# pedrosecchi67/ImmersedBoundary.jl

Hardware: AMD Instinct MI355X
Metric: Mcells*iters/s residual sweep (advection-JST-MUSCL), 2D RAE2822 (higher is better)
Workload: dtype f32

## Files before the change

### immersedboundary.jl_amd/csrc/ibh_quad2d.h

```cpp
#pragma once
#include "ibh_sweep2d.h"

namespace quad2 {

#pragma clang fp contract(fast)

typedef float v2f __attribute__((ext_vector_type(2)));
typedef float v4f __attribute__((ext_vector_type(4)));
typedef int v2i __attribute__((ext_vector_type(2)));
typedef float v4f_g __attribute__((ext_vector_type(4), aligned(4)));

#define QUAD_PITCH 20
#define QUAD_TILE (16 * QUAD_PITCH)
#define QUAD_OFF_EXT (4 * QUAD_TILE)
#define QUAD_OFF_RING (QUAD_OFF_EXT + 160)
#define QUAD_OFF_EX (QUAD_OFF_RING + 3 * 64)
#define QUAD_LDS (QUAD_OFF_EX + 64)

__device__ __forceinline__ float dpp_shr1(float old, float v) {
    return __int_as_float(__builtin_amdgcn_update_dpp(__float_as_int(old), __float_as_int(v), 0x111, 0xf, 0xf, false));
}
__device__ __forceinline__ float dpp_shl1(float old, float v) {
    return __int_as_float(__builtin_amdgcn_update_dpp(__float_as_int(old), __float_as_int(v), 0x101, 0xf, 0xf, false));
}
__device__ __forceinline__ float dpp_shl1z(float v) {
    return __int_as_float(__builtin_amdgcn_update_dpp(0, __float_as_int(v), 0x101, 0xf, 0xf, true));
}
__device__ __forceinline__ float bperm(int byte_addr, float v) {
    return __int_as_float(__builtin_amdgcn_ds_bpermute(byte_addr, __float_as_int(v)));
}
__device__ __forceinline__ float max3(float a, float b, float c) { return fmaxf(fmaxf(a, b), c); }
__device__ __forceinline__ float lds_read(const float* p) {
    float v = *p;
    asm volatile("" : "+v"(v));
    return v;
}

__device__ __forceinline__ v4f flux_half4(v4f ua, v4f ub, v4f Sa, v4f Sb, v4f Da, v4f Db, v4f Ca, v4f Cb) {
    const v4f d = ub - ua;
    const v4f gu = Sa - 0.5f * d;
    const v4f Du = Sb - 0.5f * d;
    v4f s, Df;
#pragma unroll
    for (int c = 0; c < 4; ++c) {
        s[c] = __builtin_amdgcn_fmed3f(Du[c], gu[c], 0.0f);
        Df[c] = max3(Da[c], Db[c], 1e-7f);
    }
    const v4f t16 = (Sa - Sb) * 0.0625f;
    const v4f uf = (ua + 0.5f * d) + t16;
    const v4f A = uf - Df * t16;
    const v4f Cf = 0.5f * (Ca + Cb);
    const v4f B = Df * (s - 0.5f * d);
    const v4f CA = Cf * A;
    v4f F;
#pragma unroll
    for (int c = 0; c < 4; ++c) F[c] = fmaf(fabsf(Cf[c]), B[c], CA[c]);
    return F;
}

__device__ __forceinline__ v2f flux_w2(float ua, v2f ub, float Sa, v2f Sb, float Da, v2f Db, float Ca, v2f Cb, float wa) {
    const v2f d = ub - ua;
    const v2f gu = Sa - d * wa;
    const v2f Du = Sb - d * (1.0f - wa);
    const v2f s = v2f{__builtin_amdgcn_fmed3f(Du.x, gu.x, 0.0f), __builtin_amdgcn_fmed3f(Du.y, gu.y, 0.0f)};
    const v2f t16 = (Sa - Sb) * 0.0625f;
    const v2f uf = (ua + wa * d) + t16;
    const v2f mu = d * (0.5f - wa) - t16;
    const v2f Df = v2f{max3(Da, Db.x, 1e-7f), max3(Da, Db.y, 1e-7f)};
    const v2f A = uf + Df * mu;
    const v2f Cf = Ca + wa * (Cb - Ca);
    const v2f B = Df * (s - 0.5f * d);
    const v2f CA = Cf * A;
    return v2f{fmaf(fabsf(Cf.x), B.x, CA.x), fmaf(fabsf(Cf.y), B.y, CA.y)};
}

__device__ __forceinline__ float jst(float g, float a, float rh) {
    return fmaf(fabsf(g), rh, 1e-7f) * __builtin_amdgcn_rcpf(fmaf(a, rh, 1e-7f));
}
__device__ __forceinline__ float jst_max2(float g1, float a1, float rh1, float g2, float a2, float rh2) {
    const float n1 = fmaf(fabsf(g1), rh1, 1e-7f), d1 = fmaf(a1, rh1, 1e-7f);
    const float n2 = fmaf(fabsf(g2), rh2, 1e-7f), d2 = fmaf(a2, rh2, 1e-7f);
    return fmaxf(fmaxf(n1 * d2, n2 * d1) * __builtin_amdgcn_rcpf(d1 * d2), 1e-7f);
}

template <bool HALF>
struct QuadLaneTab {
    uint32_t w[64][8];
    constexpr QuadLaneTab() : w() {
        for (int lane = 0; lane < 64; ++lane) {
            const int g = lane >> 4, t = lane & 15, tl = lane & 7, lhs = lane >> 3;
            const int ytop = HALF ? 7 : 15;
            const bool g0 = g == 0, g3 = g == 3, lr = g0 || g3, t0 = t == 0, t15 = t == ytop;
            const int bx = g0 ? 0 : g3 ? 15 : t, by = lr ? t : g == 1 ? 0 : ytop;
            const int pos_b = by * QUAD_PITCH + bx;
            const int pos_b1 = lr ? (t ^ 1) * QUAD_PITCH + bx : by * QUAD_PITCH + (t ^ 1);
            const int pos_own = t * QUAD_PITCH + 4 * g;
            const int myrow = t0 ? 0 : t15 ? 1 : 2, rowB = t0 ? 0 : 2, rowT = t15 ? 1 : 2;
            const int wrow = g == 1 ? 0 : g == 2 ? 1 : 3;
            const int eline = (lane & 31) >> 2, ee = lane & 3;
            const int epos = QUAD_OFF_EXT + eline * 20 + (ee < 2 ? ee : 16 + ee);
            const int line = QUAD_OFF_EXT + lhs * 20;
            const uint32_t f[14] = {
                (uint32_t)pos_own, (uint32_t)pos_b, (uint32_t)pos_b1, (uint32_t)(line + 2 + 2 * tl), (uint32_t)epos,
                (uint32_t)(QUAD_OFF_RING + wrow * 16 + t), (uint32_t)(QUAD_OFF_RING + myrow * 16 + 4 * g),
                (uint32_t)(QUAD_OFF_RING + rowB * 16 + 4 * g), (uint32_t)(QUAD_OFF_RING + rowT * 16 + 4 * g),
                (uint32_t)(line + 2 * tl), (uint32_t)(line + 2 * (tl & ~1)), (uint32_t)(line + 2 * (tl | 1) + 4),
                0u, 0u};
            for (int k = 0; k < 6; ++k) w[lane][k] = (4u * f[2 * k]) | ((4u * f[2 * k + 1]) << 16);
            w[lane][6] = 64u * ((g >> 1) + 2 * (t >> 3)) + 4u * (g & 1) + 8u * (t & 7);
            w[lane][7] = (uint32_t)(g0 ? -1 : g == 1 ? -8 : g == 2 ? 8 : 1);
        }
    }
};
__device__ const QuadLaneTab<false> lane_tab = QuadLaneTab<false>();
__device__ const QuadLaneTab<true> lane_tab_half = QuadLaneTab<true>();

struct QuadLane {
    float *p_own;
    float *p_b;
    float *p_b1;
    float *p_extw;
    float *p_epos;
    float *p_ringw;
    float *p_ringm;
    float *p_ringB;
    float *p_ringT;
    float *p_LbS;
    float *p_LbC;
    float *p_HbC;
    uint32_t a0off;
    int delta;
    int lane, tl, lhs;
    bool g0, g3, lr, dny, t15;
    bool active;
    float sgn;
};

template <bool HALF = false>
__device__ __forceinline__ QuadLane quad_lane(float* lds, int lane) {
    QuadLane G;
    char* const L = (char*)lds;
    const uint32_t* const tab = HALF ? lane_tab_half.w[lane] : lane_tab.w[lane];
    const uint4 w0 = *(const uint4*)(tab);
    const uint4 w1 = *(const uint4*)(tab + 4);
#define QL_LO(w) ((w) & 0xffffu)
#define QL_HI(w) ((w) >> 16)
    G.p_own = (float*)(L + QL_LO(w0.x));
    G.p_b = (float*)(L + QL_HI(w0.x));
    G.p_b1 = (float*)(L + QL_LO(w0.y));
    G.p_extw = (float*)(L + QL_HI(w0.y));
    G.p_epos = (float*)(L + QL_LO(w0.z));
    G.p_ringw = (float*)(L + QL_HI(w0.z));
    G.p_ringm = (float*)(L + QL_LO(w0.w));
    G.p_ringB = (float*)(L + QL_HI(w0.w));
    G.p_ringT = (float*)(L + QL_LO(w1.x));
    G.p_LbS = (float*)(L + QL_HI(w1.x));
    G.p_LbC = (float*)(L + QL_LO(w1.y));
    G.p_HbC = (float*)(L + QL_HI(w1.y));
#undef QL_LO
#undef QL_HI
    G.a0off = ((lane & 7) << 3) | (HALF ? 0 : ((lane & 8) << 4)) | ((lane & 16) >> 2) | ((lane & 32) << 1);
    G.delta = (int)w1.w;
    G.lane = lane;
    G.tl = lane & 7;
    G.lhs = lane >> 3;
    G.g0 = lane < 16;
    G.g3 = lane >= 48;
    G.lr = G.g0 || G.g3;
    G.dny = !G.lr;
    G.t15 = (lane & 15) == (HALF ? 7 : 15);
    G.active = !HALF || (lane & 8) == 0;
    G.sgn = lane >= 32 ? 1.0f : -1.0f;
    ((float*)(L + 4 * (QUAD_OFF_RING + 64 + 32)))[lane & 15] = 0.0f;
    ((float*)(L + 4 * (QUAD_OFF_RING + 128 + 32)))[lane & 15] = 0.5f;
    return G;
}

struct QuadTab {
    QuadDesc2 d;
    v2i hid;
    uint32_t eid;
};
struct QuadOwn {
    v4f U, CX, CY;
    uint32_t a0;
};
struct QuadHalo {
    v2f hu, hd, hc;
    float eu;
};
__device__ __forceinline__ QuadTab quad_load_tab(const QuadDesc2* __restrict__ qd, const int32_t* __restrict__ qtab,
                                                 int32_t q, int lane, const int32_t* __restrict__ qaux = nullptr) {
    QuadTab T;
    T.d = qd[q];
    const int32_t* row = qtab + (size_t)q * IBH_QROW;
    if (qaux) {
        const int32_t* aux = qaux + (size_t)q * IBH_QAUX;
        const int lhs = lane >> 3, tl = lane & 7;
        const int32_t orig = aux[32 + lhs];
        T.eid = (uint32_t)aux[lane & 31];
        const bool isC = ((T.d.cls >> (4 * lhs)) & 15u) == SIDE_COARSE;
        const bool lr = lane < 16 || lane >= 48;
        const int32_t id = orig + (lr ? 8 : 1) * (isC ? tl >> 1 : tl);
        T.hid = v2i{id, id};
        if (orig < 0) T.hid = *(const v2i*)(row + 2 * lane);
        return T;
    }
    T.hid = *(const v2i*)(row + 2 * lane);
    T.eid = (uint32_t)row[128 + (lane & 31)];
    return T;
}
__device__ __forceinline__ QuadOwn quad_load_own(const QuadLane& G, const QuadTab& T, const float* __restrict__ u,
                                                 const float* __restrict__ C, uint32_t ldc) {
    QuadOwn O;
    O.a0 = (uint32_t)T.d.base + G.a0off;
    O.U = *(const v4f_g*)((const char*)u + ((size_t)O.a0 << 2));
    O.CX = *(const v4f_g*)((const char*)C + ((size_t)O.a0 << 2));
    O.CY = *(const v4f_g*)((const char*)(C + ldc) + ((size_t)O.a0 << 2));
    return O;
}
__device__ __forceinline__ QuadHalo quad_load_halo_paired(const QuadLane& G, const QuadTab& T, const float* __restrict__ u,
                                                          const float* __restrict__ C, uint32_t ldc) {
    using blk2::ldg;
    typedef float v2f_g __attribute__((ext_vector_type(2), aligned(4)));
    auto pair = [](const float* p, int i) { return *(const v2f_g*)((const char*)p + ((size_t)(uint32_t)i << 2)); };
    QuadHalo H;
    const float* Cn = C + (G.dny ? ldc : 0u);
    const bool isF = ((T.d.cls >> (4 * G.lhs)) & 15u) == SIDE_FINE;
    const int lo = G.delta < 0 ? G.delta : 0;
    const v2f PA = pair(u, G.lr ? T.hid.x + lo : T.hid.x);
    const v2f PB = pair(u, G.lr ? T.hid.y + lo : T.hid.x + G.delta);
    const v2f PC = pair(Cn, T.hid.x);
    H.eu = ldg(u, T.eid);
    float hc1 = 0.0f;
    if (G.lr && isF) hc1 = ldg(Cn, (uint32_t)T.hid.y);
    asm volatile("" : "+v"(hc1));
    const bool first = G.g0;
    const float huA = first ? PA.y : PA.x, hdA = first ? PA.x : PA.y;
    const float huB = first ? PB.y : PB.x, hdB = first ? PB.x : PB.y;
    H.hu.x = G.lr ? huA : PA.x;
    H.hd.x = G.lr ? hdA : PB.x;
    H.hu.y = G.lr ? huB : (isF ? PA.y : PA.x);
    H.hd.y = G.lr ? hdB : (isF ? PB.y : PB.x);
    H.hc.x = PC.x;
    H.hc.y = isF ? (G.lr ? hc1 : PC.y) : PC.x;
    return H;
}

template <bool STAMP, bool STEP = false, bool HALF = false>
__device__ __forceinline__ void quad_compute(const QuadLane& G, const QuadTab& T, const QuadOwn& O, const QuadHalo& H,
                                             float* __restrict__ ud, unsigned long long* stamps, float dt = 0.0f) {
    using blk2::wave_lds_sync;
    auto stamp = [&](int k) {
        if constexpr (STAMP) {
            __builtin_amdgcn_s_waitcnt(0);
            if (stamps && G.lane == 0) stamps[k] = __builtin_amdgcn_s_memrealtime();
        }
    };
    const v4f U = O.U, CX = O.CX, CY = O.CY;
    const v2f hu = H.hu, hd = H.hd, hc = H.hc;
    const bool g0 = G.g0, g3 = G.g3, lr = G.lr, dny = G.dny, t15 = G.t15;
    const int lane = G.lane;
    const float sgn = G.sgn;
    const uint32_t ty = (T.d.cls >> (4 * G.lhs)) & 15u;
    const bool isC = ty == SIDE_COARSE, isF = ty == SIDE_FINE;
    const float qs = isC ? (1.0f / 3.0f) : isF ? (2.0f / 3.0f) : 0.5f;
    const float irt = isC ? 0.5f : isF ? 2.0f : 1.0f;
    const float rhx = T.d.rh[0], rhy = T.d.rh[1];

    *(v4f*)G.p_own = U;
    *(v4f*)(G.p_own + 3 * QUAD_TILE) = CY;
    *(v2f*)G.p_extw = hu;
    *G.p_epos = H.eu;
    wave_lds_sync();
    stamp(4);
    const float m0 = lds_read(G.p_b);
    const float m1r = lds_read(G.p_b1);
    const float m1 = isC ? m1r : m0;
    const float hm = 0.5f * (hu.x + hu.y);
    const float fix = 0.5f * (fabsf(hu.x - m0) + fabsf(hu.y - m0)) - fabsf(hm - m0);
    G.p_ringw[0] = hm;
    G.p_ringw[64] = fix;
    G.p_ringw[128] = qs;
    wave_lds_sync();
    stamp(5);

    v4f SX, SY, D;
    v4f uT;
    {
        const float uLm = bperm((lane - 16) << 2, U.w), uRp = bperm((lane + 16) << 2, U.x);
        const v4f UL = v4f{g0 ? hm : uLm, U.x, U.y, U.z};
        const v4f UR = v4f{U.y, U.z, U.w, g3 ? hm : uRp};
        const v4f qL = v4f{g0 ? qs : 0.5f, 0.5f, 0.5f, 0.5f};
        const v4f qR = v4f{0.5f, 0.5f, 0.5f, g3 ? qs : 0.5f};
        const v4f dR = UR - U, dL = U - UL;
        SX = qR * dR + qL * dL;
        const v4f gx = dR - dL;
        const v4f rM = *(const v4f*)G.p_ringm;
        const v4f rF = *(const v4f*)(G.p_ringm + 64);
        const v4f qB = *(const v4f*)(G.p_ringB + 128);
        const v4f qT = *(const v4f*)(G.p_ringT + 128);
        v4f uB;
#pragma unroll
        for (int c = 0; c < 4; ++c) {
            uB[c] = dpp_shr1(rM[c], U[c]);
            uT[c] = dpp_shl1(rM[c], U[c]);
            if constexpr (HALF) uT[c] = t15 ? rM[c] : uT[c];
        }
        const v4f dT = uT - U, dB = U - uB;
        SY = qT * dT + qB * dB;
        const v4f gy = dT - dB;
        const float fx0 = g0 ? fix : 0.0f, fx3 = g3 ? fix : 0.0f;
#pragma unroll
        for (int c = 0; c < 4; ++c) {
            float ax = fabsf(dR[c]) + fabsf(dL[c]);
            if (c == 0) ax += fx0;
            if (c == 3) ax += fx3;
            const float ay = (fabsf(dT[c]) + fabsf(dB[c])) + rF[c];
            D[c] = jst_max2(gx[c], ax, rhx, gy[c], ay, rhy);
        }
    }
    *(v4f*)(G.p_own + QUAD_TILE) = SY;
    *(v4f*)(G.p_own + 2 * QUAD_TILE) = D;

    v2f Shn, Dh;
    {
        const float ihn = (dny ? rhy : rhx) * irt, iht = (dny ? rhx : rhy) * irt;
        const v2f dm0 = m0 - hu, dm1 = m1 - hu, dde = hd - hu;
        const v2f din = 0.5f * (dm0 + dm1);
        Shn = 0.5f * dde - (1.0f - qs) * din;
        const v2f Lp = *(const v2f*)(isC ? G.p_LbC : G.p_LbS);
        const v2f Hp = *(const v2f*)(isC ? G.p_HbC : G.p_LbS + 4);
        const bool t0l = G.tl == 0, t7l = G.tl == 7;
        const v2f lo0 = v2f{(isF && !t0l) ? Lp.y : Lp.x, isF ? hu.x : Lp.x};
        const v2f lo1 = v2f{Lp.y, isF ? hu.x : Lp.y};
        const v2f hi0 = v2f{isF ? hu.y : Hp.x, Hp.x};
        const v2f hi1 = v2f{isF ? hu.y : Hp.y, (isF && !t7l) ? Hp.x : Hp.y};
        const v2f e0 = lo0 - hu, e1 = lo1 - hu, e2 = hi0 - hu, e3 = hi1 - hu;
        const v2f gn = (dm0 + dm1) + (dde + dde);
        const v2f gt = (e0 + e1) + (e2 + e3);
        const float hn = 0.5f * ihn, ht = 0.5f * iht;
#pragma unroll
        for (int k = 0; k < 2; ++k) {
            const float an = (fabsf(dm0[k]) + fabsf(dm1[k])) + 2.0f * fabsf(dde[k]);
            const float at = (fabsf(e0[k]) + fabsf(e1[k])) + (fabsf(e2[k]) + fabsf(e3[k]));
            Dh[k] = jst_max2(gn[k], an, hn, gt[k], at, ht);
        }
    }

    v4f FR, FT;
    {
        const int up = (lane + 16) << 2;
        const v4f Ub = v4f{U.y, U.z, U.w, bperm(up, U.x)};
        const v4f Sb = v4f{SX.y, SX.z, SX.w, bperm(up, SX.x)};
        const v4f Db = v4f{D.y, D.z, D.w, bperm(up, D.x)};
        const v4f Cb = v4f{CX.y, CX.z, CX.w, bperm(up, CX.x)};
        FR = flux_half4(U, Ub, SX, Sb, D, Db, CX, Cb);
        v4f St, Dt, Ct;
#pragma unroll
        for (int c = 0; c < 4; ++c) {
            St[c] = dpp_shl1z(SY[c]);
            Dt[c] = dpp_shl1z(D[c]);
            Ct[c] = dpp_shl1z(CY[c]);
        }
        FT = flux_half4(U, uT, SY, St, D, Dt, CY, Ct);
    }

    wave_lds_sync();
    stamp(6);
    float edge;
    {
        const float So_lr = g3 ? SX.w : SX.x, Do_lr = g3 ? D.w : D.x, Co_lr = g3 ? CX.w : CX.x;
        const float So_bt = lds_read(G.p_b + QUAD_TILE), Do_bt = lds_read(G.p_b + 2 * QUAD_TILE),
                    Co_bt = lds_read(G.p_b + 3 * QUAD_TILE);
        const float So = lr ? So_lr : So_bt;
        const float Do = lr ? Do_lr : Do_bt;
        const float Co = lr ? Co_lr : Co_bt;
        const v2f F = flux_w2(m0, hu, sgn * So, Shn, Do, Dh, sgn * Co, sgn * hc, qs);
        edge = sgn * (0.5f * (F.x + F.y));
    }
    G.p_ringw[QUAD_OFF_EX - QUAD_OFF_RING] = edge;
    wave_lds_sync();
    stamp(7);

    {
        const float FRm = bperm((lane - 16) << 2, FR.w);
        const v4f FL = v4f{g0 ? edge : FRm, FR.x, FR.y, FR.z};
        const v4f FRf = v4f{FR.x, FR.y, FR.z, g3 ? edge : FR.w};
        const v4f ex = *(const v4f*)(G.p_ringm + (QUAD_OFF_EX - QUAD_OFF_RING));
        v4f FB, FTf;
#pragma unroll
        for (int c = 0; c < 4; ++c) {
            FB[c] = dpp_shr1(ex[c], FT[c]);
            FTf[c] = t15 ? ex[c] : FT[c];
        }
        const v4f res = -((FRf - FL) * rhx) - ((FTf - FB) * rhy);
#ifdef Q2_NO_NT_STORE
        if (!HALF || G.active) *(v4f_g*)((char*)ud + ((size_t)O.a0 << 2)) = STEP ? U + dt * res : res;
#else
        if (!HALF || G.active) {
            if constexpr (STEP) *(v4f_g*)((char*)ud + ((size_t)O.a0 << 2)) = U + dt * res;
            else __builtin_nontemporal_store(res, (v4f_g*)((char*)ud + ((size_t)O.a0 << 2)));
        }
#endif
    }
}

template <bool STAMP, bool STEP = false, bool HALF = false>
__device__ __forceinline__ void sweep_quad(const QuadDesc2* __restrict__ qd, const int32_t* __restrict__ qtab, int32_t q,
                                           const float* __restrict__ u, const float* __restrict__ C, uint32_t ldc,
                                           float* __restrict__ ud, float* lds, int lane,
                                           unsigned long long* stamps = nullptr, float dt = 0.0f,
                                           const int32_t* __restrict__ qaux = nullptr) {
    const QuadLane G = quad_lane<HALF>(lds, lane);
    const QuadTab T = quad_load_tab(qd, qtab, q, lane, qaux);
    const QuadOwn O = quad_load_own(G, T, u, C, ldc);
    const QuadHalo H = quad_load_halo_paired(G, T, u, C, ldc);
    quad_compute<STAMP, STEP, HALF>(G, T, O, H, ud, stamps, dt);
}

#pragma clang fp contract(off)

}
```

Baseline: 123,500.

## Pad quad LDS tile with halo rows and read neighbours from LDS

The per-quad LDS tile gains two padding rows, and halo/boundary values are written into them. Vertical and horizontal neighbour values (uB, uT, UL/UR, St/Dt/Ct, FB/FT) are then read directly from LDS instead of assembled with DPP shifts, bpermutes and ring buffers with per-lane selects. Lane predicates now come from inverse_ballot masks, and the precomputed address offsets are stored pre-scaled in the lane table. The aim is fewer cross-lane ops, selects and VALU work, at the price of more LDS traffic, a larger LDS footprint and a reordered barrier.

After: 135,900, median of 6. 1.1x the previous value.

```diff
diff --git a/immersedboundary.jl_amd/csrc/ibh_quad2d.h b/immersedboundary.jl_amd/csrc/ibh_quad2d.h
--- a/immersedboundary.jl_amd/csrc/ibh_quad2d.h
+++ b/immersedboundary.jl_amd/csrc/ibh_quad2d.h
@@ -11,20 +11,16 @@
 typedef float v4f_g __attribute__((ext_vector_type(4), aligned(4)));
 
 #define QUAD_PITCH 20
-#define QUAD_TILE (16 * QUAD_PITCH)
+#define QUAD_TILE (18 * QUAD_PITCH)
 #define QUAD_OFF_EXT (4 * QUAD_TILE)
 #define QUAD_OFF_RING (QUAD_OFF_EXT + 160)
-#define QUAD_OFF_EX (QUAD_OFF_RING + 3 * 64)
-#define QUAD_LDS (QUAD_OFF_EX + 64)
+#define QUAD_LDS (QUAD_OFF_RING + 2 * 64)
 
 __device__ __forceinline__ float dpp_shr1(float old, float v) {
     return __int_as_float(__builtin_amdgcn_update_dpp(__float_as_int(old), __float_as_int(v), 0x111, 0xf, 0xf, false));
 }
 __device__ __forceinline__ float dpp_shl1(float old, float v) {
     return __int_as_float(__builtin_amdgcn_update_dpp(__float_as_int(old), __float_as_int(v), 0x101, 0xf, 0xf, false));
-}
-__device__ __forceinline__ float dpp_shl1z(float v) {
-    return __int_as_float(__builtin_amdgcn_update_dpp(0, __float_as_int(v), 0x101, 0xf, 0xf, true));
 }
 __device__ __forceinline__ float bperm(int byte_addr, float v) {
     return __int_as_float(__builtin_amdgcn_ds_bpermute(byte_addr, __float_as_int(v)));
@@ -92,34 +88,38 @@
             const int ytop = HALF ? 7 : 15;
             const bool g0 = g == 0, g3 = g == 3, lr = g0 || g3, t0 = t == 0, t15 = t == ytop;
             const int bx = g0 ? 0 : g3 ? 15 : t, by = lr ? t : g == 1 ? 0 : ytop;
-            const int pos_b = by * QUAD_PITCH + bx;
-            const int pos_b1 = lr ? (t ^ 1) * QUAD_PITCH + bx : by * QUAD_PITCH + (t ^ 1);
-            const int pos_own = t * QUAD_PITCH + 4 * g;
+            const int pos_b = (by + 1) * QUAD_PITCH + bx;
+            const int pos_b1 = lr ? ((t ^ 1) + 1) * QUAD_PITCH + bx : (by + 1) * QUAD_PITCH + (t ^ 1);
+            const int pos_up = t * QUAD_PITCH + 4 * g;
+            const int pos_hm = g0 ? (t + 1) * QUAD_PITCH - 1 : g3 ? (t + 1) * QUAD_PITCH + 16 : g == 1 ? t : (ytop + 2) * QUAD_PITCH + t;
+            const int pos_exw = g == 1 ? t : g == 2 ? (ytop + 1) * QUAD_PITCH + t : 17 * QUAD_PITCH + 19;
             const int myrow = t0 ? 0 : t15 ? 1 : 2, rowB = t0 ? 0 : 2, rowT = t15 ? 1 : 2;
             const int wrow = g == 1 ? 0 : g == 2 ? 1 : 3;
             const int eline = (lane & 31) >> 2, ee = lane & 3;
             const int epos = QUAD_OFF_EXT + eline * 20 + (ee < 2 ? ee : 16 + ee);
             const int line = QUAD_OFF_EXT + lhs * 20;
-            const uint32_t f[14] = {
-                (uint32_t)pos_own, (uint32_t)pos_b, (uint32_t)pos_b1, (uint32_t)(line + 2 + 2 * tl), (uint32_t)epos,
+            const uint32_t f[12] = {
+                (uint32_t)pos_up, (uint32_t)pos_b, (uint32_t)pos_b1, (uint32_t)epos,
                 (uint32_t)(QUAD_OFF_RING + wrow * 16 + t), (uint32_t)(QUAD_OFF_RING + myrow * 16 + 4 * g),
                 (uint32_t)(QUAD_OFF_RING + rowB * 16 + 4 * g), (uint32_t)(QUAD_OFF_RING + rowT * 16 + 4 * g),
-                (uint32_t)(line + 2 * tl), (uint32_t)(line + 2 * (tl & ~1)), (uint32_t)(line + 2 * (tl | 1) + 4),
-                0u, 0u};
+                (uint32_t)(line + 2 * tl), (uint32_t)(line + 2 * (tl & ~1)), (uint32_t)pos_hm, (uint32_t)pos_exw};
             for (int k = 0; k < 6; ++k) w[lane][k] = (4u * f[2 * k]) | ((4u * f[2 * k + 1]) << 16);
-            w[lane][6] = 64u * ((g >> 1) + 2 * (t >> 3)) + 4u * (g & 1) + 8u * (t & 7);
-            w[lane][7] = (uint32_t)(g0 ? -1 : g == 1 ? -8 : g == 2 ? 8 : 1);
+            w[lane][6] = 4u * (64u * ((g >> 1) + (HALF ? 0 : 2 * (t >> 3))) + 4u * (g & 1) + 8u * (t & 7));
+            w[lane][7] = (uint32_t)(g0 ? -1 : g == 1 ? -8 : g == 2 ? 8 : 0);
         }
     }
 };
 __device__ const QuadLaneTab<false> lane_tab = QuadLaneTab<false>();
 __device__ const QuadLaneTab<true> lane_tab_half = QuadLaneTab<true>();
 
+#define QL_MASK(m) __builtin_amdgcn_inverse_ballot_w64(m)
+
 struct QuadLane {
-    float *p_own;
+    float *p_up;
+    float *p_hm;
+    float *p_exw;
     float *p_b;
     float *p_b1;
-    float *p_extw;
     float *p_epos;
     float *p_ringw;
     float *p_ringm;
@@ -127,11 +127,11 @@
     float *p_ringT;
     float *p_LbS;
     float *p_LbC;
-    float *p_HbC;
-    uint32_t a0off;
-    int delta;
-    int lane, tl, lhs;
-    bool g0, g3, lr, dny, t15;
+    uint32_t a0off4;
+    int offB;
+    int lane;
+    bool g0, g3, lr, dny;
+    bool tl0, tl7;
     bool active;
     float sgn;
 };
@@ -145,45 +145,44 @@
     const uint4 w1 = *(const uint4*)(tab + 4);
 #define QL_LO(w) ((w) & 0xffffu)
 #define QL_HI(w) ((w) >> 16)
-    G.p_own = (float*)(L + QL_LO(w0.x));
+    G.p_up = (float*)(L + QL_LO(w0.x));
     G.p_b = (float*)(L + QL_HI(w0.x));
     G.p_b1 = (float*)(L + QL_LO(w0.y));
-    G.p_extw = (float*)(L + QL_HI(w0.y));
-    G.p_epos = (float*)(L + QL_LO(w0.z));
-    G.p_ringw = (float*)(L + QL_HI(w0.z));
-    G.p_ringm = (float*)(L + QL_LO(w0.w));
-    G.p_ringB = (float*)(L + QL_HI(w0.w));
-    G.p_ringT = (float*)(L + QL_LO(w1.x));
-    G.p_LbS = (float*)(L + QL_HI(w1.x));
-    G.p_LbC = (float*)(L + QL_LO(w1.y));
-    G.p_HbC = (float*)(L + QL_HI(w1.y));
+    G.p_epos = (float*)(L + QL_HI(w0.y));
+    G.p_ringw = (float*)(L + QL_LO(w0.z));
+    G.p_ringm = (float*)(L + QL_HI(w0.z));
+    G.p_ringB = (float*)(L + QL_LO(w0.w));
+    G.p_ringT = (float*)(L + QL_HI(w0.w));
+    G.p_LbS = (float*)(L + QL_LO(w1.x));
+    G.p_LbC = (float*)(L + QL_HI(w1.x));
+    G.p_hm = (float*)(L + QL_LO(w1.y));
+    G.p_exw = (float*)(L + QL_HI(w1.y));
 #undef QL_LO
 #undef QL_HI
-    G.a0off = ((lane & 7) << 3) | (HALF ? 0 : ((lane & 8) << 4)) | ((lane & 16) >> 2) | ((lane & 32) << 1);
-    G.delta = (int)w1.w;
+    G.sgn = QL_MASK(0xffffffff00000000ull) ? 1.0f : -1.0f;
+    G.a0off4 = w1.z;
+    G.offB = (int)w1.w;
     G.lane = lane;
-    G.tl = lane & 7;
-    G.lhs = lane >> 3;
-    G.g0 = lane < 16;
-    G.g3 = lane >= 48;
-    G.lr = G.g0 || G.g3;
-    G.dny = !G.lr;
-    G.t15 = (lane & 15) == (HALF ? 7 : 15);
-    G.active = !HALF || (lane & 8) == 0;
-    G.sgn = lane >= 32 ? 1.0f : -1.0f;
-    ((float*)(L + 4 * (QUAD_OFF_RING + 64 + 32)))[lane & 15] = 0.0f;
-    ((float*)(L + 4 * (QUAD_OFF_RING + 128 + 32)))[lane & 15] = 0.5f;
+    G.g0 = QL_MASK(0x000000000000ffffull);
+    G.g3 = QL_MASK(0xffff000000000000ull);
+    G.lr = QL_MASK(0xffff00000000ffffull);
+    G.dny = QL_MASK(0x0000ffffffff0000ull);
+    G.tl0 = QL_MASK(0x0101010101010101ull);
+    G.tl7 = QL_MASK(0x8080808080808080ull);
+    G.active = QL_MASK(HALF ? 0x00ff00ff00ff00ffull : ~0ull);
+    ((float*)(L + 4 * (QUAD_OFF_RING + 32)))[lane & 15] = 0.0f;
+    ((float*)(L + 4 * (QUAD_OFF_RING + 64 + 32)))[lane & 15] = 0.5f;
     return G;
 }
 
 struct QuadTab {
     QuadDesc2 d;
+    uint32_t ty;
     v2i hid;
     uint32_t eid;
 };
 struct QuadOwn {
     v4f U, CX, CY;
-    uint32_t a0;
 };
 struct QuadHalo {
     v2f hu, hd, hc;
@@ -193,14 +192,15 @@
                                                  int32_t q, int lane, const int32_t* __restrict__ qaux = nullptr) {
     QuadTab T;
     T.d = qd[q];
+    T.ty = (T.d.cls >> ((lane >> 1) & 28)) & 15u;
     const int32_t* row = qtab + (size_t)q * IBH_QROW;
     if (qaux) {
         const int32_t* aux = qaux + (size_t)q * IBH_QAUX;
         const int lhs = lane >> 3, tl = lane & 7;
         const int32_t orig = aux[32 + lhs];
         T.eid = (uint32_t)aux[lane & 31];
-        const bool isC = ((T.d.cls >> (4 * lhs)) & 15u) == SIDE_COARSE;
-        const bool lr = lane < 16 || lane >= 48;
+        const bool isC = T.ty == SIDE_COARSE;
+        const bool lr = QL_MASK(0xffff00000000ffffull);
         const int32_t id = orig + (lr ? 8 : 1) * (isC ? tl >> 1 : tl);
         T.hid = v2i{id, id};
         if (orig < 0) T.hid = *(const v2i*)(row + 2 * lane);
@@ -210,13 +210,14 @@
     T.eid = (uint32_t)row[128 + (lane & 31)];
     return T;
 }
+__device__ __forceinline__ size_t quad_base4(const QuadTab& T) { return (size_t)(uint32_t)T.d.base << 2; }
 __device__ __forceinline__ QuadOwn quad_load_own(const QuadLane& G, const QuadTab& T, const float* __restrict__ u,
                                                  const float* __restrict__ C, uint32_t ldc) {
     QuadOwn O;
-    O.a0 = (uint32_t)T.d.base + G.a0off;
-    O.U = *(const v4f_g*)((const char*)u + ((size_t)O.a0 << 2));
-    O.CX = *(const v4f_g*)((const char*)C + ((size_t)O.a0 << 2));
-    O.CY = *(const v4f_g*)((const char*)(C + ldc) + ((size_t)O.a0 << 2));
+    const size_t b4 = quad_base4(T);
+    O.U = *(const v4f_g*)((const char*)u + b4 + G.a0off4);
+    O.CX = *(const v4f_g*)((const char*)C + b4 + G.a0off4);
+    O.CY = *(const v4f_g*)((const char*)(C + ldc) + b4 + G.a0off4);
     return O;
 }
 __device__ __forceinline__ QuadHalo quad_load_halo_paired(const QuadLane& G, const QuadTab& T, const float* __restrict__ u,
@@ -226,22 +227,20 @@
     auto pair = [](const float* p, int i) { return *(const v2f_g*)((const char*)p + ((size_t)(uint32_t)i << 2)); };
     QuadHalo H;
     const float* Cn = C + (G.dny ? ldc : 0u);
-    const bool isF = ((T.d.cls >> (4 * G.lhs)) & 15u) == SIDE_FINE;
-    const int lo = G.delta < 0 ? G.delta : 0;
-    const v2f PA = pair(u, G.lr ? T.hid.x + lo : T.hid.x);
-    const v2f PB = pair(u, G.lr ? T.hid.y + lo : T.hid.x + G.delta);
+    const bool isF = T.ty == SIDE_FINE;
+    const v2f PA = pair(u, T.hid.x - (int)G.g0);
+    const v2f PB = pair(u, (G.lr ? T.hid.y : T.hid.x) + G.offB);
     const v2f PC = pair(Cn, T.hid.x);
     H.eu = ldg(u, T.eid);
     float hc1 = 0.0f;
     if (G.lr && isF) hc1 = ldg(Cn, (uint32_t)T.hid.y);
     asm volatile("" : "+v"(hc1));
-    const bool first = G.g0;
-    const float huA = first ? PA.y : PA.x, hdA = first ? PA.x : PA.y;
-    const float huB = first ? PB.y : PB.x, hdB = first ? PB.x : PB.y;
-    H.hu.x = G.lr ? huA : PA.x;
-    H.hd.x = G.lr ? hdA : PB.x;
-    H.hu.y = G.lr ? huB : (isF ? PA.y : PA.x);
-    H.hd.y = G.lr ? hdB : (isF ? PB.y : PB.x);
+    const bool dF = G.dny && isF;
+    const float a = dF ? PA.y : PA.x;
+    H.hu.x = G.g0 ? PA.y : PA.x;
+    H.hd.x = G.g0 ? PA.x : (G.g3 ? PA.y : PB.x);
+    H.hu.y = G.g0 ? PB.y : (G.g3 ? PB.x : a);
+    H.hd.y = (G.g3 || dF) ? PB.y : PB.x;
     H.hc.x = PC.x;
     H.hc.y = isF ? (G.lr ? hc1 : PC.y) : PC.x;
     return H;
@@ -259,18 +258,19 @@
     };
     const v4f U = O.U, CX = O.CX, CY = O.CY;
     const v2f hu = H.hu, hd = H.hd, hc = H.hc;
-    const bool g0 = G.g0, g3 = G.g3, lr = G.lr, dny = G.dny, t15 = G.t15;
+    const bool g0 = G.g0, g3 = G.g3, lr = G.lr, dny = G.dny;
     const int lane = G.lane;
     const float sgn = G.sgn;
-    const uint32_t ty = (T.d.cls >> (4 * G.lhs)) & 15u;
+    const uint32_t ty = T.ty;
     const bool isC = ty == SIDE_COARSE, isF = ty == SIDE_FINE;
     const float qs = isC ? (1.0f / 3.0f) : isF ? (2.0f / 3.0f) : 0.5f;
     const float irt = isC ? 0.5f : isF ? 2.0f : 1.0f;
     const float rhx = T.d.rh[0], rhy = T.d.rh[1];
 
-    *(v4f*)G.p_own = U;
-    *(v4f*)(G.p_own + 3 * QUAD_TILE) = CY;
-    *(v2f*)G.p_extw = hu;
+    float* const p_own = G.p_up + QUAD_PITCH;
+    *(v4f*)p_own = U;
+    *(v4f*)(p_own + 3 * QUAD_TILE) = CY;
+    *(v2f*)(G.p_LbS + 2) = hu;
     *G.p_epos = H.eu;
     wave_lds_sync();
     stamp(4);
@@ -279,34 +279,28 @@
     const float m1 = isC ? m1r : m0;
     const float hm = 0.5f * (hu.x + hu.y);
     const float fix = 0.5f * (fabsf(hu.x - m0) + fabsf(hu.y - m0)) - fabsf(hm - m0);
-    G.p_ringw[0] = hm;
-    G.p_ringw[64] = fix;
-    G.p_ringw[128] = qs;
+    *G.p_hm = hm;
+    G.p_ringw[0] = fix;
+    G.p_ringw[64] = qs;
     wave_lds_sync();
     stamp(5);
 
     v4f SX, SY, D;
     v4f uT;
     {
-        const float uLm = bperm((lane - 16) << 2, U.w), uRp = bperm((lane + 16) << 2, U.x);
-        const v4f UL = v4f{g0 ? hm : uLm, U.x, U.y, U.z};
-        const v4f UR = v4f{U.y, U.z, U.w, g3 ? hm : uRp};
+        const v4f UL = v4f{p_own[-1], U.x, U.y, U.z};
+        const v4f UR = v4f{U.y, U.z, U.w, p_own[4]};
         const v4f qL = v4f{g0 ? qs : 0.5f, 0.5f, 0.5f, 0.5f};
         const v4f qR = v4f{0.5f, 0.5f, 0.5f, g3 ? qs : 0.5f};
         const v4f dR = UR - U, dL = U - UL;
-        SX = qR * dR + qL * dL;
+#pragma unroll
+        for (int c = 0; c < 4; ++c) SX[c] = fmaf(qR[c], dR[c], qL[c] * dL[c]);
         const v4f gx = dR - dL;
-        const v4f rM = *(const v4f*)G.p_ringm;
-        const v4f rF = *(const v4f*)(G.p_ringm + 64);
-        const v4f qB = *(const v4f*)(G.p_ringB + 128);
-        const v4f qT = *(const v4f*)(G.p_ringT + 128);
-        v4f uB;
-#pragma unroll
-        for (int c = 0; c < 4; ++c) {
-            uB[c] = dpp_shr1(rM[c], U[c]);
-            uT[c] = dpp_shl1(rM[c], U[c]);
-            if constexpr (HALF) uT[c] = t15 ? rM[c] : uT[c];
-        }
+        const v4f rF = *(const v4f*)G.p_ringm;
+        const v4f qB = *(const v4f*)(G.p_ringB + 64);
+        const v4f qT = *(const v4f*)(G.p_ringT + 64);
+        const v4f uB = *(const v4f*)G.p_up;
+        uT = *(const v4f*)(G.p_up + 2 * QUAD_PITCH);
         const v4f dT = uT - U, dB = U - uB;
         SY = qT * dT + qB * dB;
         const v4f gy = dT - dB;
@@ -320,8 +314,8 @@
             D[c] = jst_max2(gx[c], ax, rhx, gy[c], ay, rhy);
         }
     }
-    *(v4f*)(G.p_own + QUAD_TILE) = SY;
-    *(v4f*)(G.p_own + 2 * QUAD_TILE) = D;
+    *(v4f*)(p_own + QUAD_TILE) = SY;
+    *(v4f*)(p_own + 2 * QUAD_TILE) = D;
 
     v2f Shn, Dh;
     {
@@ -330,8 +324,8 @@
         const v2f din = 0.5f * (dm0 + dm1);
         Shn = 0.5f * dde - (1.0f - qs) * din;
         const v2f Lp = *(const v2f*)(isC ? G.p_LbC : G.p_LbS);
-        const v2f Hp = *(const v2f*)(isC ? G.p_HbC : G.p_LbS + 4);
-        const bool t0l = G.tl == 0, t7l = G.tl == 7;
+        const v2f Hp = *(const v2f*)((isC ? G.p_LbC + 2 : G.p_LbS) + 4);
+        const bool t0l = G.tl0, t7l = G.tl7;
         const v2f lo0 = v2f{(isF && !t0l) ? Lp.y : Lp.x, isF ? hu.x : Lp.x};
         const v2f lo1 = v2f{Lp.y, isF ? hu.x : Lp.y};
         const v2f hi0 = v2f{isF ? hu.y : Hp.x, Hp.x};
@@ -348,6 +342,8 @@
         }
     }
 
+    wave_lds_sync();
+    stamp(6);
     v4f FR, FT;
     {
         const int up = (lane + 16) << 2;
@@ -356,30 +352,24 @@
         const v4f Db = v4f{D.y, D.z, D.w, bperm(up, D.x)};
         const v4f Cb = v4f{CX.y, CX.z, CX.w, bperm(up, CX.x)};
         FR = flux_half4(U, Ub, SX, Sb, D, Db, CX, Cb);
-        v4f St, Dt, Ct;
-#pragma unroll
-        for (int c = 0; c < 4; ++c) {
-            St[c] = dpp_shl1z(SY[c]);
-            Dt[c] = dpp_shl1z(D[c]);
-            Ct[c] = dpp_shl1z(CY[c]);
-        }
+        const v4f St = *(const v4f*)(p_own + QUAD_TILE + QUAD_PITCH);
+        const v4f Dt = *(const v4f*)(p_own + 2 * QUAD_TILE + QUAD_PITCH);
+        const v4f Ct = *(const v4f*)(p_own + 3 * QUAD_TILE + QUAD_PITCH);
         FT = flux_half4(U, uT, SY, St, D, Dt, CY, Ct);
     }
-
-    wave_lds_sync();
-    stamp(6);
+    *(v4f*)p_own = FT;
+
     float edge;
     {
-        const float So_lr = g3 ? SX.w : SX.x, Do_lr = g3 ? D.w : D.x, Co_lr = g3 ? CX.w : CX.x;
-        const float So_bt = lds_read(G.p_b + QUAD_TILE), Do_bt = lds_read(G.p_b + 2 * QUAD_TILE),
+        const float So_lr = g3 ? SX.w : SX.x, Co_lr = g3 ? CX.w : CX.x;
+        const float So_bt = lds_read(G.p_b + QUAD_TILE), Do = lds_read(G.p_b + 2 * QUAD_TILE),
                     Co_bt = lds_read(G.p_b + 3 * QUAD_TILE);
         const float So = lr ? So_lr : So_bt;
-        const float Do = lr ? Do_lr : Do_bt;
         const float Co = lr ? Co_lr : Co_bt;
         const v2f F = flux_w2(m0, hu, sgn * So, Shn, Do, Dh, sgn * Co, sgn * hc, qs);
         edge = sgn * (0.5f * (F.x + F.y));
     }
-    G.p_ringw[QUAD_OFF_EX - QUAD_OFF_RING] = edge;
+    *G.p_exw = edge;
     wave_lds_sync();
     stamp(7);
 
@@ -387,20 +377,16 @@
         const float FRm = bperm((lane - 16) << 2, FR.w);
         const v4f FL = v4f{g0 ? edge : FRm, FR.x, FR.y, FR.z};
         const v4f FRf = v4f{FR.x, FR.y, FR.z, g3 ? edge : FR.w};
-        const v4f ex = *(const v4f*)(G.p_ringm + (QUAD_OFF_EX - QUAD_OFF_RING));
-        v4f FB, FTf;
-#pragma unroll
-        for (int c = 0; c < 4; ++c) {
-            FB[c] = dpp_shr1(ex[c], FT[c]);
-            FTf[c] = t15 ? ex[c] : FT[c];
-        }
+        const v4f FB = *(const v4f*)G.p_up;
+        const v4f FTf = *(const v4f*)p_own;
         const v4f res = -((FRf - FL) * rhx) - ((FTf - FB) * rhy);
+        float* const out = (float*)((char*)ud + quad_base4(T) + G.a0off4);
 #ifdef Q2_NO_NT_STORE
-        if (!HALF || G.active) *(v4f_g*)((char*)ud + ((size_t)O.a0 << 2)) = STEP ? U + dt * res : res;
+        if (!HALF || G.active) *(v4f_g*)out = STEP ? U + dt * res : res;
 #else
         if (!HALF || G.active) {
-            if constexpr (STEP) *(v4f_g*)((char*)ud + ((size_t)O.a0 << 2)) = U + dt * res;
-            else __builtin_nontemporal_store(res, (v4f_g*)((char*)ud + ((size_t)O.a0 << 2)));
+            if constexpr (STEP) *(v4f_g*)out = U + dt * res;
+            else __builtin_nontemporal_store(res, (v4f_g*)out);
         }
 #endif
     }
```
